# beenotung/bpe-tokenizer

Hardware: NVIDIA B200
Metric: mergeUntil merges/sec (higher is better)
Workload: dtype u32

## Files before the change

### bpe_tokenizer_b200/csrc/bpe_b200.cu

```cuda
#include "../../include/bpe_b200.h"

#include <algorithm>
#include <cstdarg>
#include <cstdio>
#include <cstdlib>
#include <chrono>
#include <cstring>
#include <functional>
#include <string>
#include <unordered_map>
#include <vector>

#include "encode_kernels.cuh"
#include "encode_lanes.cuh"
#include "encode_dp.cuh"
#include "train_kernels.cuh"
#include "mg_kernels.cuh"
#include "round_kernels.cuh"
#include "text_kernels.cuh"

using namespace bpe;

namespace {

// ... 87 lines not shown

struct EncodeScratch {
  DevBuf<int32_t> out_tmp;
  DevBuf<uint32_t> out_len;
  DevBuf<uint64_t> out_off;
  DevBuf<uint32_t> g_tok, g_nxt, g_prv, g_rk, g_sel;
  DevBuf<uint32_t> range_first, tile_sums;
  DevBuf<uint64_t> tile_off;
  DevBuf<uint32_t> flags;
  DevBuf<uint16_t> dp_last;
  DevBuf<unsigned long long> dp_cursor;
};

struct bpe_engine {
  int device = 0;
  int sm_count = 148;
  cudaStream_t stream = nullptr, own_stream = nullptr;
  std::string err;
  bool profiling = false;
  cudaEvent_t ev0 = nullptr, ev1 = nullptr;

  DevBuf<uint32_t> slots;
  uint64_t n_slots = 0;
  std::vector<int64_t> doc_off{0};
  uint64_t live_tokens = 0;

  std::vector<int32_t> h_len16;
  DevBuf<uint32_t> d_len16;
  int32_t n_tokens = 0;

  std::vector<int32_t> h_merges;
  bool mt_dirty = true;
  DevBuf<unsigned long long> d_mt;
  DevBuf<uint32_t> d_minlr;
  uint32_t mt_cap = 0;
  bool lt_dirty = true;
  DevBuf<uint4> d_lt;
  DevBuf<uint2> d_lt_dense;
  DevBuf<uint16_t> d_rule_c;
  uint32_t lt_cap = 0;
  int32_t lt_c_affine = -1;
  bool dp_dirty = true, dp_ok = false;
  DevBuf<unsigned long long> d_dfa;
  DevBuf<uint32_t> d_split;
  DevBuf<uint16_t> d_tok_len, d_shorter;
  bool dp_attr_set = false;
  uint32_t dp_alpha = 0;
  int enc_dp = 0;
  int enc_lmax = 32;
  int enc_lmax_forced = 0;
  int enc_force_old = 0;

  bool index_valid = false;
  uint32_t tbl_cap = 0;
  DevBuf<uint32_t> t_ent;
  DevBuf<uint32_t> u_ent;
  DevBuf<uint32_t> pool;
  DevBuf<DevState> d_st;
  DevState* h_st = nullptr;
  DevBuf<Best> partials;
  DevBuf<uint32_t> partial_keys;
  DevBuf<SiteRec> sites, sites2;
  DevBuf<uint32_t> newslots;
  DevBuf<uint32_t> nd;
  DevBuf<uint32_t> hot;
  bool hot_valid = false;
  uint32_t hot_max_length = 0;
  uint32_t hot_thresh = 0;
  uint32_t hot_limit = 0;
  DevBuf<uint32_t> cands;
  DevBuf<MergeRec> dev_log;
  DevBuf<unsigned long long> barrier;
  int loop_blocks = 0;
  DevBuf<unsigned long long> r_cells;
  DevBuf<uint32_t> r_slotrows, r_lists;
  DevBuf<SiteRec> r_bsites;
  DevBuf<uint4> r_gp;
  DevBuf<uint32_t> r_gk;
  DevBuf<RoundState> r_state;
  DevBuf<unsigned long long> r_gcells;
  DevBuf<uint32_t> r_glists;
  int round_blocks = 0;
  int host_loop = 0;
  int scan_mode = 0;

  int mg_rank = 0, mg_world = 1;
  void* mg_mailbox = nullptr;
  size_t mg_mailbox_bytes = 0;
  void* mg_peer[MG_MAX_WORLD] = {};
  bool mg_connected = false;
  bool mg_counts_global = false;
  uint32_t mg_inbox_stride = 0, mg_tie_cap = 0;
  DevBuf<int32_t> mg_dlt;
  DevBuf<uint32_t> mg_mark, mg_touched, mg_tie_sorted, mg_export_n, mg_newpair;
  int mg_loop_blocks = 0;
  unsigned long long mg_epoch = 0, mg_tie_epoch = 0;

  DevBuf<int32_t> d_cpmap;
  DevBuf<uint32_t> d_firstpos;
  DevBuf<uint8_t> x_text;
  DevBuf<uint32_t> x_tilecnt;
  DevBuf<uint64_t> x_tileoff;
  DevBuf<unsigned long long> x_counts;
  DevBuf<uint32_t> x_doccnt;
  DevBuf<uint64_t> x_docoff;

  DevBuf<int32_t> x_ids, x_out, x_tvi;
  DevBuf<int64_t> x_off, x_ooff, x_ooff2, x_bad;
  DevBuf<unsigned long long> x_flag;
  std::vector<int64_t> h_rel;
  EncodeScratch x_scratch;
  EncodeScratch dev_scratch;
  uint32_t lanes_attr_set = 0;
  cudaStream_t s_in = nullptr, s_out = nullptr;
  cudaEvent_t ev_in[3] = {nullptr, nullptr, nullptr}, ev_done = nullptr, ev_res[2] = {nullptr, nullptr};
  unsigned long long* h_pipe = nullptr;
  PinBuf<int64_t> h_in_off, h_out_off, h_bad;
  int64_t enc_chunk = 128ll << 20;

  DevBuf<int32_t> stage_ids;
  DevBuf<int64_t> stage_off;

  bpe_stats stats{};

  PairTable table() const {
    PairTable t;
    const size_t fs = (TBL_STRIDE == 1) ? (size_t)tbl_cap : 1;
    t.keys.p = t_ent.p;
    t.cnt.p = t_ent.p + fs;
    t.occ_start.p = t_ent.p + 2 * fs;
    t.occ_len.p = t_ent.p + 3 * fs;
    t.occ_fill.p = t_ent.p + 4 * fs;
    t.mask = tbl_cap - 1;
    t.shift = 32 - ilog2(tbl_cap);
    return t;
  }
  int grid(int per_sm = 4) const { return sm_count * per_sm; }
};

namespace {

int fail(bpe_engine* e, int code, const char* fmt, ...) {
  char buf[512];
  va_list ap;
  va_start(ap, fmt);
  vsnprintf(buf, sizeof buf, fmt, ap);
  va_end(ap);
  if (e) e->err = buf;
  return code;
}

#define CK(call)                                                                                              \
  do {                                                                                                        \
    cudaError_t _err = (call);                                                                                \
    if (_err != cudaSuccess)                                                                                  \
      return fail(e, _err == cudaErrorMemoryAllocation ? BPE_E_NOMEM : BPE_E_CUDA, "%s:%d %s: %s", __FILE__, \
                  __LINE__, #call, cudaGetErrorString(_err));                                                 \
  } while (0)

#define CKL()                                \
  do {                                       \
    e->stats.kernel_launches++;              \
    CK(cudaGetLastError());                  \
  } while (0)

#define TRY(call)             \
  do {                        \
    int _rc = (call);         \
    if (_rc != BPE_OK) return _rc; \
  } while (0)

int fetch_state(bpe_engine* e) {
  CK(cudaMemcpyAsync(e->h_st, e->d_st.p, sizeof(DevState), cudaMemcpyDeviceToHost, e->stream));
  CK(cudaStreamSynchronize(e->stream));
  return BPE_OK;
}

int check_dev_err(bpe_engine* e) {
  uint32_t f = e->h_st->err & ~ERR_HOT_OVERFLOW;
  if (!f) return BPE_OK;
  if (f & ERR_POOL_FULL) return fail(e, BPE_E_INTERNAL, "occurrence pool exhausted (flags 0x%x)", f);
  if (f & ERR_MISSING_KEY) return fail(e, BPE_E_INTERNAL, "pair missing from the table (flags 0x%x)", f);
  if (f & ERR_SPAN_OVERFLOW) return fail(e, BPE_E_DOMAIN, "token span exceeds 2^29 positions");
  return fail(e, BPE_E_INTERNAL, "device error flags 0x%x", f);
}

int sync_len16(bpe_engine* e) {
  size_t n = e->h_len16.size();
  CK(e->d_len16.reserve(std::max<size_t>(n + 1024, 4096), 0, e->stream, 2.0));
  if (n) {
    std::vector<uint32_t> tmp(e->h_len16.begin(), e->h_len16.end());
    CK(cudaMemcpyAsync(e->d_len16.p, tmp.data(), n * sizeof(uint32_t), cudaMemcpyHostToDevice, e->stream));
    CK(cudaStreamSynchronize(e->stream));
  }
  return BPE_OK;
}

__global__ void k_init_table(uint4* __restrict__ ent, uint64_t cap) {
  uint64_t stride = (uint64_t)gridDim.x * blockDim.x;
  for (uint64_t i = (uint64_t)blockIdx.x * blockDim.x + threadIdx.x; i < cap; i += stride) {
    ent[2 * i] = make_uint4(EMPTY_KEY, 0u, 0u, 0u);
    ent[2 * i + 1] = make_uint4(0u, 0u, 0u, 0u);
  }
}

int alloc_table(bpe_engine* e, uint32_t cap) {
  CK(e->t_ent.reserve((size_t)cap * (TBL_STRIDE == 1 ? 5 : TBL_STRIDE)));
  e->tbl_cap = cap;
  if (TBL_STRIDE == 1) {
    CK(cudaMemsetAsync(e->t_ent.p, 0xFF, (size_t)cap * 4, e->stream));
    CK(cudaMemsetAsync(e->t_ent.p + cap, 0, (size_t)cap * 16, e->stream));
  } else {
    k_init_table<<<e->grid(8), 256, 0, e->stream>>>(reinterpret_cast<uint4*>(e->t_ent.p), (uint64_t)cap);
    CKL();
  }
  if (e->mg_world > 1) {
    CK(e->mg_dlt.reserve(cap));
    CK(cudaMemsetAsync(e->mg_dlt.p, 0, (size_t)cap * 4, e->stream));
  }
  return BPE_OK;
}

__global__ void k_rehash(PairTable src, PairTable dst, DevState* st) {
  uint32_t cap = src.mask + 1;
  for (uint32_t i = blockIdx.x * blockDim.x + threadIdx.x; i < cap; i += gridDim.x * blockDim.x) {
    uint32_t key = src.keys[i];
    if (key == EMPTY_KEY) continue;
    uint32_t h = (key * 0x9E3779B1u) >> dst.shift;
    for (;;) {
      uint32_t old = atomicCAS(dst.keys + h, EMPTY_KEY, key);
      if (old == EMPTY_KEY) break;
      h = (h + 1) & dst.mask;
    }
    dst.cnt[h] = src.cnt[i];
    dst.occ_start[h] = src.occ_start[i];
    dst.occ_len[h] = src.occ_len[i];
    dst.occ_fill[h] = src.occ_fill[i];
  }
}

int grow_table(bpe_engine* e, uint32_t new_cap) {
  PairTable old = e->table();
  std::swap(e->t_ent, e->u_ent);
  TRY(alloc_table(e, new_cap));
  k_rehash<<<e->grid(), 256, 0, e->stream>>>(old, e->table(), e->d_st.p);
  CKL();
  CK(cudaStreamSynchronize(e->stream));
  e->hot_valid = false;
  return BPE_OK;
}

int build_index(bpe_engine* e) {
  e->index_valid = false;
  e->hot_valid = false;
  if (!e->h_st) CK(cudaHostAlloc((void**)&e->h_st, sizeof(DevState), cudaHostAllocDefault));
  CK(e->d_st.reserve(1));
  CK(e->partials.reserve((size_t)e->grid(8)));
  if (!e->nd.p) CK(e->nd.reserve((size_t)ND_ROWS * ND_STRIDE));
  CK(cudaMemsetAsync(e->nd.p, 0, (size_t)ND_ROWS * ND_STRIDE * 4, e->stream));
  TRY(sync_len16(e));
  uint64_t n = e->n_slots;
  if (n >= 0xFFFFFFF0ull) return fail(e, BPE_E_DOMAIN, "corpus of %llu positions exceeds the 2^32 engine limit", (unsigned long long)n);
  uint64_t pool_need = 3 * n + 1024;
  if (pool_need > 0xFFFFFFF0ull) pool_need = 0xFFFFFFF0ull;
  CK(e->pool.reserve((size_t)pool_need));
  uint64_t t2 = (uint64_t)e->n_tokens * (uint64_t)e->n_tokens;
  uint32_t cap = pow2_at_least(std::min<uint64_t>(std::max<uint64_t>(2 * std::min(n, t2), 1u << 16), 1u << 24));
  {
    if (!e->ev0) {
      CK(cudaEventCreate(&e->ev0));
      CK(cudaEventCreate(&e->ev1));
    }
    CK(cudaEventRecord(e->ev0, e->stream));
  }
  for (;;) {
    TRY(alloc_table(e, cap));
    DevState init{};
    init.live_tokens = e->live_tokens;
    init.tie_pos = ~0ull;
    init.mg_epoch = e->mg_epoch;
    init.mg_tie_epoch = e->mg_tie_epoch;
    CK(cudaMemcpyAsync(e->d_st.p, &init, sizeof init, cudaMemcpyHostToDevice, e->stream));
    CK(cudaStreamSynchronize(e->stream));
    if (n) {
      k_hist<<<e->grid(4), K1_THREADS, 0, e->stream>>>(e->slots.p, (uint32_t)n, e->table(), e->d_st.p);
      CKL();
    }
    TRY(fetch_state(e));
    if (e->h_st->err & ERR_TABLE_FULL) {
      if (cap >= 0x80000000u) return fail(e, BPE_E_NOMEM, "pair table cannot grow further");
      cap <<= 2;
      continue;
    }
    TRY(check_dev_err(e));
    if ((uint64_t)e->h_st->n_keys * 2 > cap && cap < 0x80000000u) {
      cap <<= 1;
      continue;
    }
    break;
  }
  if (n) {
    k_alloc_lists<<<e->grid(4), 256, 0, e->stream>>>(e->table(), e->d_st.p, (uint32_t)e->pool.cap);
    CKL();
    int k1b_per_sm = 8;
    if (const char* v = getenv("BPE_K1B_PER_SM")) k1b_per_sm = std::max(1, std::min(atoi(v), 8));
    k_scatter<<<e->grid(k1b_per_sm), K1_THREADS, 0, e->stream>>>(e->slots.p, (uint32_t)n, e->table(), e->pool.p, e->d_st.p);
    CKL();
  }
  CK(cudaEventRecord(e->ev1, e->stream));
  TRY(fetch_state(e));
  TRY(check_dev_err(e));
  float ms = 0;
  CK(cudaEventElapsedTime(&ms, e->ev0, e->ev1));
  e->stats.ms_index_build += ms;
  e->stats.index_builds++;
  e->index_valid = true;
  e->mg_counts_global = false;
  return BPE_OK;
}

int ensure_index(bpe_engine* e) {
  if (e->index_valid) return BPE_OK;
  return build_index(e);
}

constexpr uint32_t HOT_TARGET = 1u << 15;

int rebuild_hot(bpe_engine* e, uint32_t max_length, bool* any) {
  PairTable t = e->table();
  CK(cudaMemsetAsync(&e->d_st.p->bins[0], 0, sizeof(uint32_t) * 36, e->stream));
  k_count_bins<<<e->grid(4), 256, 0, e->stream>>>(t, e->d_len16.p, max_length, e->d_st.p);
  CKL();
  TRY(fetch_state(e));
  uint64_t acc = 0;
  int pick = 0;
  for (int k = 32; k >= 1; k--) {
    uint64_t nk = e->h_st->bins[k];
    if (acc + nk > HOT_TARGET && acc > 0) break;
    acc += nk;
    if (nk) pick = k;
    if (acc > HOT_TARGET) break;
  }
  *any = pick != 0;
  e->hot_valid = false;
  if (!pick) return BPE_OK;
  int lo = pick;
  while (lo > 1 && e->h_st->bins[lo - 1] == 0) lo--;
  uint32_t thresh = 1u << (lo - 1);
  CK(e->hot.reserve(std::max<size_t>((size_t)acc * 2 + 4096 + 2 * (size_t)BPE_MAX_TOKENS, 1u << 18)));
  e->h_st->hot_n = 0;
  e->h_st->hot_thresh = thresh;
  uint32_t two[2] = {0, thresh};
  CK(cudaMemcpyAsync(&e->d_st.p->hot_n, two, sizeof two, cudaMemcpyHostToDevice, e->stream));
  k_build_hot<<<e->grid(4), 256, 0, e->stream>>>(t, e->d_len16.p, max_length, e->hot.p, (uint32_t)e->hot.cap, e->d_st.p);
  CKL();
  e->hot_thresh = thresh;
  e->hot_limit = (uint32_t)std::min<uint64_t>(std::max<uint64_t>(4ull * HOT_TARGET, 2 * acc + 4096), 0xFFFFFFF0u);
  e->hot_max_length = max_length;
  e->hot_valid = true;
  e->stats.hot_rebuilds++;
  return BPE_OK;
}

int run_argmax(bpe_engine* e, uint32_t max_length, int use_hot) {
  PairTable t = e->table();
  int blocks = use_hot ? e->sm_count : e->grid(4);
  k_argmax<<<blocks, AM_THREADS, 0, e->stream>>>(t, e->d_len16.p, max_length, use_hot, e->hot.p, e->partials.p, e->d_st.p);
  CKL();
  TRY(fetch_state(e));
  TRY(check_dev_err(e));
  if (e->h_st->best_primary && e->h_st->best_mult > 1 && !(use_hot && e->h_st->best_cnt < e->hot_thresh)) {
    uint32_t mult = e->h_st->best_mult;
    CK(e->cands.reserve(std::max<size_t>(mult, 1024), 0, e->stream, 2.0));
    k_collect_cands<<<blocks, 256, 0, e->stream>>>(t, e->d_len16.p, max_length, use_hot, e->hot.p, e->cands.p, (uint32_t)e->cands.cap, e->d_st.p);
    CKL();
    k_tie_break<<<std::min<uint32_t>(mult, (uint32_t)e->grid(4)), 256, 0, e->stream>>>(e->slots.p, (uint32_t)e->n_slots, t, e->pool.p, e->cands.p, e->d_st.p);
    CKL();
    k_tie_finish<<<1, 32, 0, e->stream>>>(t, e->d_st.p);
    CKL();
    TRY(fetch_state(e));
    TRY(check_dev_err(e));
    e->stats.tie_breaks++;
  }
  return BPE_OK;
}

ApplyArgs apply_args(bpe_engine* e) {
  ApplyArgs A;
  A.slots = e->slots.p;
  A.n = (uint32_t)e->n_slots;
  A.t = e->table();
  A.pool = e->pool.p;
  A.st = e->d_st.p;
  A.sites = e->sites.p;
  A.sites_cap = (uint32_t)std::min<size_t>(e->sites.cap, 0xFFFFFFFFu);
  A.newslots = e->newslots.p;
  A.nd = e->nd.p;
  A.newpair = nullptr;
  A.newpair_cap = 0;
  A.new_cap = (uint32_t)std::min<size_t>(e->newslots.cap, 0xFFFFFFFFu);
  A.len16 = e->d_len16.p;
  A.scan_mode = e->scan_mode;
  A.dlt = nullptr;
  A.touched = nullptr;
  A.touched_cap = 0;
  for (int q = 0; q < 8; q++) A.push[q] = nullptr;
  A.push_world = 0;
  A.push_cap = 0;
  return A;
}

int run_apply(bpe_engine* e, uint32_t a, uint32_t b, uint32_t c, uint32_t bound) {
  uint64_t keys_after = (uint64_t)e->h_st->n_keys + std::min<uint64_t>(2ull * bound + 2, 2ull * ((uint64_t)e->n_tokens + 1) + 2);
  if (keys_after * 2 > e->tbl_cap) {
    uint64_t want = keys_after * 5 / 2;
    if (want > 0x80000000ull) want = 0x80000000ull;
    if (keys_after * 2 > pow2_at_least(want)) return fail(e, BPE_E_NOMEM, "pair table cannot grow further");
    TRY(grow_table(e, pow2_at_least(want)));
  }
  uint64_t pool_after = (uint64_t)e->h_st->pool_cursor + 2ull * bound;
  if (pool_after > e->pool.cap) {
    if (pool_after > 0xFFFFFFF0ull) return fail(e, BPE_E_DOMAIN, "occurrence pool exceeds 2^32 cells");
    CK(e->pool.reserve((size_t)pool_after, e->h_st->pool_cursor, e->stream, 1.5));
  }
  CK(e->sites.reserve(std::max<size_t>(bound, 4096), 0, e->stream, 2.0));
  CK(e->newslots.reserve(std::max<size_t>(2ull * bound + 2, 8192), 0, e->stream, 2.0));
  if ((size_t)c + 1 > e->d_len16.cap) CK(e->d_len16.reserve((size_t)c + 1, (size_t)c, e->stream, 2.0));
  PairTable t = e->table();
  uint32_t work = e->scan_mode ? (uint32_t)e->n_slots : bound;
  int blocks = (int)std::min<uint64_t>((uint64_t)e->grid(8), std::max<uint64_t>(1, (work + 255) / 256));
  ApplyArgs A = apply_args(e);
  k_sites<<<blocks, 256, 0, e->stream>>>(A, a, b, c);
  CKL();
  int blocks2 = (int)std::min<uint64_t>((uint64_t)e->grid(8), std::max<uint64_t>(1, (2ull * bound + 255) / 256));
  k_alloc_new<<<blocks2, 256, 0, e->stream>>>(A, c, e->hot_max_length, e->hot_valid ? 1 : 0, e->hot.p, (uint32_t)e->hot.cap, (uint32_t)e->pool.cap);
  CKL();
  int blocks3 = (int)std::min<uint64_t>((uint64_t)e->grid(8), std::max<uint64_t>(1, ((uint64_t)bound + 255) / 256));
  k_apply<<<blocks3, 256, 0, e->stream>>>(A, a, b, c);
  CKL();
  e->h_len16.push_back(e->h_len16[a] + e->h_len16[b]);
  e->h_merges.push_back((int32_t)a);
  e->h_merges.push_back((int32_t)b);
  e->h_merges.push_back((int32_t)c);
  e->mt_dirty = e->lt_dirty = e->dp_dirty = true;
  e->n_tokens++;
  e->stats.merges_applied++;
  return BPE_OK;
}

int ensure_merge_table(bpe_engine* e) {
  if (!e->mt_dirty && e->d_mt.p) return BPE_OK;
  size_t m = e->h_merges.size() / 3;
  uint32_t cap = pow2_at_least(std::max<size_t>(4 * m, 1024));
  std::vector<unsigned long long> h(cap, MT_EMPTY);
  int shift = 32 - ilog2(cap);
  for (size_t r = 0; r < m; r++) {
    uint32_t a = (uint32_t)e->h_merges[3 * r], b = (uint32_t)e->h_merges[3 * r + 1], c = (uint32_t)e->h_merges[3 * r + 2];
    uint32_t key = pair_key(a, b);
    uint32_t i = (key * 0x9E3779B1u) >> shift;
    bool dup = false;
    while (h[i] != MT_EMPTY) {
      if ((uint32_t)(h[i] >> 32) == key) {
        dup = true;
        break;
      }
      i = (i + 1) & (cap - 1);
    }
    if (!dup) h[i] = ((unsigned long long)key << 32) | ((unsigned long long)(uint32_t)r << 16) | c;
  }
  std::vector<uint32_t> minlr((size_t)std::max(e->n_tokens, 1), 0xFFFFFFFFu);
  for (size_t r = 0; r < m; r++) {
    uint32_t a = (uint32_t)e->h_merges[3 * r], b = (uint32_t)e->h_merges[3 * r + 1];
    if (a >= minlr.size() || b >= minlr.size()) return fail(e, BPE_E_INVALID, "merge %zu refers to a token outside the table", r);
    uint32_t rr = (uint32_t)std::min<size_t>(r, 0xFFFE);
    if ((minlr[a] >> 16) > rr) minlr[a] = (minlr[a] & 0xFFFFu) | (rr << 16);
    if ((minlr[b] & 0xFFFFu) > rr) minlr[b] = (minlr[b] & 0xFFFF0000u) | rr;
  }
  CK(e->d_minlr.reserve(minlr.size()));
  CK(cudaMemcpyAsync(e->d_minlr.p, minlr.data(), minlr.size() * 4, cudaMemcpyHostToDevice, e->stream));
  CK(e->d_mt.reserve(cap));
  CK(cudaMemcpyAsync(e->d_mt.p, h.data(), (size_t)cap * 8, cudaMemcpyHostToDevice, e->stream));
  CK(cudaStreamSynchronize(e->stream));
  e->mt_cap = cap;
  e->mt_dirty = false;
  return BPE_OK;
}

struct LaneEnt {
  uint16_t rk = 0xFFFF, c = 0, rs = 0xFFFF, ls = 0xFFFF;
};

int build_lane_entries(bpe_engine* e, const std::vector<int32_t>& merges, int32_t n_tokens, std::unordered_map<uint32_t, LaneEnt>& M,
                       std::vector<uint16_t>& rule_c) {
  size_t m = merges.size() / 3;
  if (m > EL_MAX_RANK + 1) return fail(e, BPE_E_DOMAIN, "merge list too long");
  const int32_t nt = std::max(n_tokens, 1);
  M.clear();
  M.reserve(m * 3 + 16);
  std::vector<int32_t> def_a((size_t)nt, -1), def_b((size_t)nt, -1);
  std::vector<uint8_t> first(m, 0);
  rule_c.assign(std::max<size_t>(m, 1), 0);
  for (size_t r = 0; r < m; r++) {
    int32_t a = merges[3 * r], b = merges[3 * r + 1], c = merges[3 * r + 2];
    if (a < 0 || b < 0 || c < 0 || a >= nt || b >= nt || c >= nt)
      return fail(e, BPE_E_INVALID, "merge %zu refers to a token outside the table", r);
    rule_c[r] = (uint16_t)c;
    if (def_a[c] < 0 && a < c && b < c) {
      def_a[c] = a;
      def_b[c] = b;
    } else if (def_a[c] >= 0 && (def_a[c] != a || def_b[c] != b)) {
      return fail(e, BPE_E_INVALID, "token %d is produced by two different merges", c);
    }
    LaneEnt& x = M[pair_key((uint32_t)a, (uint32_t)b)];
    if (x.rk == 0xFFFF) {
      x.rk = (uint16_t)r;
      x.c = (uint16_t)c;
      first[r] = 1;
    }
  }
  for (size_t r = 0; r < m; r++) {
    if (!first[r]) continue;
    int32_t a = merges[3 * r], b = merges[3 * r + 1];
    for (int32_t u = a;;) {
      LaneEnt& x = M[pair_key((uint32_t)u, (uint32_t)b)];
      if (x.rs > r) x.rs = (uint16_t)r;
      if (def_a[u] < 0) break;
      u = def_b[u];
    }
    for (int32_t w = b;;) {
      LaneEnt& x = M[pair_key((uint32_t)a, (uint32_t)w)];
      if (x.ls > r) x.ls = (uint16_t)r;
      if (def_a[w] < 0) break;
      w = def_a[w];
    }
  }
  return BPE_OK;
}

int ensure_lane_tables(bpe_engine* e) {
  if (!e->lt_dirty && e->d_lt.p) return BPE_OK;
  size_t m = e->h_merges.size() / 3;
  std::unordered_map<uint32_t, LaneEnt> M;
  std::vector<uint16_t> rule_c;
  TRY(build_lane_entries(e, e->h_merges, e->n_tokens, M, rule_c));
  uint32_t cap = pow2_at_least(std::max<size_t>(2 * M.size(), 1024));
  std::vector<uint4> h(cap, make_uint4(EMPTY_KEY, EL_NONE, 0xFFFFFFFFu, 0));
  std::vector<uint2> dense((size_t)EL_DENSE * EL_DENSE, make_uint2(EL_NONE, 0xFFFFFFFFu));
  int shift = 32 - ilog2(cap);
  for (auto& kv : M) {
    uint32_t key = kv.first;
    const LaneEnt& x = kv.second;
    uint32_t y = (uint32_t)x.rk | ((uint32_t)x.c << 16), z = (uint32_t)x.rs | ((uint32_t)x.ls << 16);
    uint32_t a = key >> 16, b = key & 0xFFFFu;
    if (a < (uint32_t)EL_DENSE && b < (uint32_t)EL_DENSE) dense[a * EL_DENSE + b] = make_uint2(y, z);
    uint32_t i = (key * 0x9E3779B1u) >> shift;
    while (h[i].x != EMPTY_KEY) i = (i + 1) & (cap - 1);
    h[i] = make_uint4(key, y, z, 0);
  }
  CK(e->d_lt.reserve(cap));
  CK(cudaMemcpyAsync(e->d_lt.p, h.data(), (size_t)cap * sizeof(uint4), cudaMemcpyHostToDevice, e->stream));
  CK(e->d_lt_dense.reserve(dense.size()));
  CK(cudaMemcpyAsync(e->d_lt_dense.p, dense.data(), dense.size() * sizeof(uint2), cudaMemcpyHostToDevice, e->stream));
  CK(e->d_rule_c.reserve(rule_c.size()));
  CK(cudaMemcpyAsync(e->d_rule_c.p, rule_c.data(), rule_c.size() * sizeof(uint16_t), cudaMemcpyHostToDevice, e->stream));
  CK(cudaStreamSynchronize(e->stream));
  e->lt_cap = cap;
  e->lt_c_affine = m ? (int32_t)rule_c[0] : 0;
  for (size_t r = 0; r < m; r++)
    if ((int64_t)rule_c[r] != (int64_t)rule_c[0] + (int64_t)r) e->lt_c_affine = -1;
  e->lt_dirty = false;
  return BPE_OK;
}

int ensure_dp_tables(bpe_engine* e) {
  if (!e->dp_dirty) return BPE_OK;
  e->dp_dirty = false;
  e->dp_ok = false;
  const size_t m = e->h_merges.size() / 3;
  const int64_t n_tok = e->n_tokens;
  const int64_t A = n_tok - (int64_t)m;
  if (A <= 0 || A > 4096 || n_tok > 0xFFF0) return BPE_OK;
  std::vector<uint32_t> split((size_t)n_tok), off((size_t)n_tok + 1, 0);
  std::vector<uint16_t> tok_len((size_t)n_tok, 1);
  for (int64_t t = 0; t < A; t++) split[(size_t)t] = (uint32_t)t | ((uint32_t)t << 16);
  for (size_t r = 0; r < m; r++) {
    const int64_t a = e->h_merges[3 * r], b = e->h_merges[3 * r + 1], c = e->h_merges[3 * r + 2];
    if (c != A + (int64_t)r || a < 0 || b < 0 || a >= c || b >= c) return BPE_OK;
    const uint32_t L = (uint32_t)tok_len[(size_t)a] + tok_len[(size_t)b];
    if (L > 0xFFF0u) return BPE_OK;
    tok_len[(size_t)c] = (uint16_t)L;
    split[(size_t)c] = (uint32_t)a | ((uint32_t)b << 16);
  }
  for (int64_t t = 0; t < n_tok; t++) off[(size_t)t + 1] = off[(size_t)t] + tok_len[(size_t)t];
  if (off[(size_t)n_tok] > (64u << 20)) return BPE_OK;
  std::vector<uint16_t> text(off[(size_t)n_tok]);
  for (int64_t t = 0; t < A; t++) text[off[(size_t)t]] = (uint16_t)t;
  for (size_t r = 0; r < m; r++) {
    const size_t a = (size_t)e->h_merges[3 * r], b = (size_t)e->h_merges[3 * r + 1], c = (size_t)e->h_merges[3 * r + 2];
    std::copy(text.begin() + off[a], text.begin() + off[a + 1], text.begin() + off[c]);
    std::copy(text.begin() + off[b], text.begin() + off[b + 1], text.begin() + off[c] + tok_len[a]);
  }
  std::unordered_map<uint64_t, uint32_t> child;
  child.reserve(text.size() * 2);
  std::vector<uint16_t> node_tok(1, (uint16_t)DP_NONE);
  std::vector<uint32_t> node_of((size_t)n_tok), parent(1, 0);
  std::vector<uint16_t> pch(1, 0);
  for (int64_t t = 0; t < n_tok; t++) {
    uint32_t v = 0;
    for (uint32_t i = off[(size_t)t]; i < off[(size_t)t + 1]; i++) {
// ... 1960 lines not shown
```

### bpe_tokenizer_b200/csrc/train_kernels.cuh

```cuda
#pragma once
#include "common.cuh"

namespace bpe {

struct DevState {
  uint32_t n_keys;
  uint32_t pool_cursor;
  uint32_t err;
  uint32_t hot_n;
  uint32_t hot_thresh;
  uint32_t n_sites[2];
  uint32_t n_new[2];
  uint32_t n_cand;
  uint32_t blocks_done;
  unsigned long long best_primary;
  uint32_t best_slot;
  uint32_t best_mult;
  uint32_t best_a, best_b, best_cnt;
  uint32_t list_len;
  unsigned long long tie_pos;
  unsigned long long live_tokens;
  unsigned long long _unused_barrier;
  uint32_t n_tokens;
  uint32_t iters_done;
  uint32_t status;
  uint32_t tie_breaks;
  unsigned long long sites_total;
  uint32_t snap_n_keys, snap_pool_cursor, snap_hot_n, snap_err;
  unsigned long long prof_ns[8];
  uint32_t bins[36];
  unsigned long long mg_epoch;
  unsigned long long mg_tie_epoch;
  uint32_t n_touched[2];
  uint32_t n_out;
  uint32_t n_newpair;
  uint32_t mg_abort;
  unsigned long long mg_prof_ns[12];
  alignas(16) uint32_t g_vals[8];
  unsigned long long fine_ns[12];
  unsigned long long bucket_ns[32][4];
};

constexpr uint32_t LOOP_RUNNING = 0, LOOP_DONE = 1, LOOP_NEED_REBUILD = 2, LOOP_NEED_HOST = 3, LOOP_EMPTY = 4,
                   LOOP_ERROR = 5, LOOP_LIMIT = 6;

struct SiteRec {
  uint32_t p;
  uint32_t lpos;
  uint32_t lslot;
  uint32_t rslot;
};

struct MergeRec {
  int32_t a, b, c, reserved;
  long long weight;
};

__device__ __forceinline__ unsigned long long make_primary(uint32_t cnt, uint32_t a, uint32_t b) {
  return ((unsigned long long)cnt << 20) | (unsigned long long)(0xFFFFFu - (a + b));
}

__device__ __forceinline__ uint32_t lane_id() { return threadIdx.x & 31u; }

__global__ void k_ingest_ids(const int32_t* __restrict__ ids, uint32_t* __restrict__ slots, uint64_t n,
                             uint32_t max_id, uint32_t* __restrict__ err) {
  uint64_t i4 = (uint64_t)blockIdx.x * blockDim.x + threadIdx.x;
  uint64_t stride = (uint64_t)gridDim.x * blockDim.x;
  uint64_t n4 = n >> 2;
  bool aligned = ((((uintptr_t)ids) | ((uintptr_t)slots)) & 15) == 0;
  uint32_t bad = 0;
  if (aligned) {
    for (uint64_t i = i4; i < n4; i += stride) {
      int4 v = __ldg(reinterpret_cast<const int4*>(ids) + i);
      bad |= ((uint32_t)v.x >= max_id) | ((uint32_t)v.y >= max_id) | ((uint32_t)v.z >= max_id) | ((uint32_t)v.w >= max_id);
      reinterpret_cast<uint4*>(slots)[i] = make_uint4((uint32_t)v.x, (uint32_t)v.y, (uint32_t)v.z, (uint32_t)v.w);
    }
    for (uint64_t i = (n4 << 2) + i4; i < n; i += stride) {
      uint32_t v = (uint32_t)ids[i];
      bad |= v >= max_id;
      slots[i] = v;
    }
  } else {
    for (uint64_t i = i4; i < n; i += stride) {
      uint32_t v = (uint32_t)ids[i];
      bad |= v >= max_id;
      slots[i] = v;
    }
  }
  if (bad) atomicOr(err, 1u);
}

__global__ void k_validate_ids(const uint32_t* __restrict__ slots, uint64_t n, uint32_t max_id, uint32_t* __restrict__ err) {
  uint64_t stride = (uint64_t)gridDim.x * blockDim.x;
  uint32_t bad = 0;
  for (uint64_t i = (uint64_t)blockIdx.x * blockDim.x + threadIdx.x; i < n; i += stride) bad |= slots[i] >= max_id;
  if (bad) atomicOr(err, 1u);
}

__global__ void k_mark_docstarts(uint32_t* __restrict__ slots, const int64_t* __restrict__ doc_off, int64_t n_docs,
                                 int64_t base) {
  int64_t d = (int64_t)blockIdx.x * blockDim.x + threadIdx.x;
  int64_t stride = (int64_t)gridDim.x * blockDim.x;
  for (; d < n_docs; d += stride) {
    int64_t s = doc_off[d], e = doc_off[d + 1];
    if (e > s) slots[base + s] |= DOCSTART;
  }
}

constexpr int K1_THREADS = 256;
constexpr int K1_SMEM_SLOTS = 2048;
constexpr int K1_MAX_PROBE = 8;
#ifndef BPE_K1B_CHUNK_LOG
#define BPE_K1B_CHUNK_LOG 16
#endif
constexpr uint32_t K1B_CHUNK = 1u << BPE_K1B_CHUNK_LOG;

struct SmemHist {
  uint32_t key[K1_SMEM_SLOTS];
  uint32_t a[K1_SMEM_SLOTS];
  uint32_t b[K1_SMEM_SLOTS];
};

__device__ __forceinline__ int sh_slot(SmemHist& sh, uint32_t key, bool insert) {
  uint32_t h = (key * 0x9E3779B1u) >> (32 - 11);
#pragma unroll 1
  for (int probe = 0; probe < K1_MAX_PROBE; probe++) {
    uint32_t k = sh.key[h];
    if (k == EMPTY_KEY) {
      if (!insert) return -1;
      uint32_t old = atomicCAS(&sh.key[h], EMPTY_KEY, key);
      k = (old == EMPTY_KEY) ? key : old;
    }
    if (k == key) return (int)h;
    h = (h + 1) & (K1_SMEM_SLOTS - 1);
  }
  return -1;
}

__device__ __forceinline__ bool edge_at(const uint32_t* __restrict__ slots, uint32_t n, uint32_t p, uint32_t w,
                                        uint32_t wnext_hint, uint32_t* key, uint32_t* counted) {
  if (!slot_is_id(w)) return false;
  uint32_t a = slot_val(w);
  int b;
  if (slot_is_id(wnext_hint)) {
    b = (wnext_hint & DOCSTART) ? NOTOK : (int)slot_val(wnext_hint);
  } else {
    uint32_t q;
    b = right_token(slots, n, p, &q);
  }
  if (b == NOTOK) return false;
  *key = pair_key(a, (uint32_t)b);
  if (counted) {
    *counted = 1;
    if ((uint32_t)b == a) *counted = (run_left(slots, p, w, (int)a) & 1u) ? 0u : 1u;
  }
  return true;
}

__device__ __forceinline__ void load_group(const uint32_t* __restrict__ slots, uint32_t n, uint32_t g, uint32_t v[5]) {
  uint32_t p0 = g << 2;
  if (p0 + 4 <= n) {
    uint4 q = ld_slots4(slots + p0);
    v[0] = q.x; v[1] = q.y; v[2] = q.z; v[3] = q.w;
  } else {
#pragma unroll
    for (int j = 0; j < 4; j++) v[j] = (p0 + j < n) ? ld_slot(slots + p0 + j) : mk_hole();
  }
  v[4] = (p0 + 4 < n) ? ld_slot(slots + p0 + 4) : (DOCSTART);
}

__global__ void __launch_bounds__(K1_THREADS) k_hist(const uint32_t* __restrict__ slots, uint32_t n, PairTable t,
                                                      DevState* st) {
  __shared__ SmemHist sh;
  for (int i = threadIdx.x; i < K1_SMEM_SLOTS; i += K1_THREADS) {
    sh.key[i] = EMPTY_KEY;
    sh.a[i] = 0;
    sh.b[i] = 0;
  }
  __syncthreads();
  uint32_t n4 = (n + 3) >> 2;
  uint32_t per_block = (n4 + gridDim.x - 1) / gridDim.x;
  uint32_t g_begin = blockIdx.x * per_block;
  uint32_t g_end = min(n4, g_begin + per_block);
  for (uint32_t g = g_begin + threadIdx.x; g < g_end; g += K1_THREADS) {
    uint32_t p0 = g << 2;
    uint32_t v[5];
    load_group(slots, n, g, v);
#pragma unroll
    for (int j = 0; j < 4; j++) {
      uint32_t key, counted;
      if (p0 + j < n && edge_at(slots, n, p0 + j, v[j], v[j + 1], &key, &counted)) {
        int h = sh_slot(sh, key, true);
        if (h >= 0) {
          atomicAdd(&sh.a[h], 1u);
          if (!counted) atomicAdd(&sh.b[h], 1u);
        } else {
          uint32_t gs = tbl_find_or_insert(t, key, &st->n_keys);
          if (gs == NOSLOT) {
            atomicOr(&st->err, ERR_TABLE_FULL);
          } else {
            if (counted) atomicAdd(t.cnt + gs, 1u);
            atomicAdd(t.occ_len + gs, 1u);
          }
        }
      }
    }
  }
  __syncthreads();
  uint32_t n_ins = 0;
  for (int i = threadIdx.x; i < K1_SMEM_SLOTS; i += K1_THREADS) {
    uint32_t key = sh.key[i];
    if (key == EMPTY_KEY) continue;
    bool ins;
    uint32_t gs = tbl_find_or_insert_ex(t, key, &ins);
    if (gs == NOSLOT) {
      atomicOr(&st->err, ERR_TABLE_FULL);
      continue;
    }
    n_ins += ins ? 1u : 0u;
    if (sh.a[i] != sh.b[i]) atomicAdd(t.cnt + gs, sh.a[i] - sh.b[i]);
    if (sh.a[i]) atomicAdd(t.occ_len + gs, sh.a[i]);
  }
#pragma unroll
  for (int o = 16; o > 0; o >>= 1) n_ins += __shfl_xor_sync(0xFFFFFFFFu, n_ins, o);
  if ((threadIdx.x & 31) == 0 && n_ins) atomicAdd(&st->n_keys, n_ins);
}

__global__ void k_alloc_lists(PairTable t, DevState* st, uint32_t pool_cap) {
  uint32_t cap = t.mask + 1;
  for (uint32_t i = blockIdx.x * blockDim.x + threadIdx.x; i < cap; i += gridDim.x * blockDim.x) {
    if (t.keys[i] == EMPTY_KEY) continue;
    uint32_t len = t.occ_len[i];
    t.occ_fill[i] = 0;
    if (len == 0) continue;
    uint32_t start = atomicAdd(&st->pool_cursor, len);
    if (start > pool_cap || len > pool_cap - start) atomicOr(&st->err, ERR_POOL_FULL);
    t.occ_start[i] = start;
  }
}

__global__ void __launch_bounds__(K1_THREADS) k_scatter(const uint32_t* __restrict__ slots, uint32_t n, PairTable t,
                                                         uint32_t* __restrict__ pool, DevState* st) {
  __shared__ SmemHist sh;
  uint32_t n_chunks = (n + K1B_CHUNK - 1) / K1B_CHUNK;
  for (uint32_t chunk = blockIdx.x; chunk < n_chunks; chunk += gridDim.x) {
    for (int i = threadIdx.x; i < K1_SMEM_SLOTS; i += K1_THREADS) {
      sh.key[i] = EMPTY_KEY;
      sh.a[i] = 0;
    }
    __syncthreads();
    uint32_t g_begin = chunk * (K1B_CHUNK >> 2);
    uint32_t g_end = min((n + 3) >> 2, g_begin + (K1B_CHUNK >> 2));
    for (uint32_t g = g_begin + threadIdx.x; g < g_end; g += K1_THREADS) {
      uint32_t p0 = g << 2;
      uint32_t v[5];
      load_group(slots, n, g, v);
#pragma unroll
      for (int j = 0; j < 4; j++) {
        uint32_t key;
        if (p0 + j < n && edge_at(slots, n, p0 + j, v[j], v[j + 1], &key, nullptr)) {
          int h = sh_slot(sh, key, true);
          if (h >= 0) atomicAdd(&sh.a[h], 1u);
        }
      }
    }
    __syncthreads();
    for (int i = threadIdx.x; i < K1_SMEM_SLOTS; i += K1_THREADS) {
      uint32_t key = sh.key[i];
      if (key == EMPTY_KEY) continue;
      uint32_t gs = tbl_find(t, key);
      if (gs == NOSLOT) {
        atomicOr(&st->err, ERR_MISSING_KEY);
        sh.b[i] = NOPOS;
      } else {
        sh.b[i] = t.occ_start[gs] + atomicAdd(t.occ_fill + gs, sh.a[i]);
      }
      sh.a[i] = 0;
    }
    __syncthreads();
    for (uint32_t g = g_begin + threadIdx.x; g < g_end; g += K1_THREADS) {
      uint32_t p0 = g << 2;
      uint32_t v[5];
      load_group(slots, n, g, v);
#pragma unroll
      for (int j = 0; j < 4; j++) {
        uint32_t key;
        if (p0 + j < n && edge_at(slots, n, p0 + j, v[j], v[j + 1], &key, nullptr)) {
          int h = sh_slot(sh, key, false);
          if (h >= 0) {
            uint32_t base = sh.b[h];
            if (base != NOPOS) pool[base + atomicAdd(&sh.a[h], 1u)] = p0 + j;
          } else {
            uint32_t gs = tbl_find(t, key);
            if (gs == NOSLOT) atomicOr(&st->err, ERR_MISSING_KEY);
            else pool[t.occ_start[gs] + atomicAdd(t.occ_fill + gs, 1u)] = p0 + j;
          }
        }
      }
    }
    __syncthreads();
  }
}

struct Best {
  unsigned long long primary;
  uint32_t slot;
  uint32_t mult;
};

__device__ __forceinline__ Best best_merge(Best x, Best y) {
  if (x.primary > y.primary) return x;
  if (y.primary > x.primary) return y;
  Best r;
  r.primary = x.primary;
  r.slot = min(x.slot, y.slot);
  r.mult = x.mult + y.mult;
  return r;
}

__device__ __forceinline__ Best best_warp_reduce(Best v) {
#pragma unroll
  for (int o = 16; o > 0; o >>= 1) {
    Best w;
    w.primary = __shfl_xor_sync(0xFFFFFFFFu, v.primary, o);
    w.slot = __shfl_xor_sync(0xFFFFFFFFu, v.slot, o);
    w.mult = __shfl_xor_sync(0xFFFFFFFFu, v.mult, o);
    v = best_merge(v, w);
  }
  return v;
}

__device__ __forceinline__ Best best_block_reduce(Best v, Best* s_best) {
  v = best_warp_reduce(v);
  __syncthreads();
  if (lane_id() == 0) s_best[threadIdx.x >> 5] = v;
  __syncthreads();
  uint32_t nw = blockDim.x >> 5;
  Best u = (lane_id() < nw) ? s_best[lane_id()] : Best{0ull, NOSLOT, 0};
  u = best_warp_reduce(u);
  return u;
}

__device__ __forceinline__ unsigned long long slot_primary(const PairTable& t, const uint32_t* len16, uint32_t s,
                                                           uint32_t max_length) {
  uint32_t key = t.keys[s];
  if (key == EMPTY_KEY) return 0ull;
  uint32_t c = t.cnt[s];
  if (c == 0) return 0ull;
  uint32_t a = key >> 16, b = key & 0xFFFFu;
  if (max_length && len16[a] + len16[b] > max_length) return 0ull;
  return make_primary(c, a, b);
}

__device__ __forceinline__ unsigned long long slot_primary_k(const PairTable& t, const uint32_t* len16, uint32_t s, uint32_t max_length,
                                                             uint32_t* key_out) {
  uint32_t key = t.keys[s];
  *key_out = key;
  if (key == EMPTY_KEY) return 0ull;
  uint32_t c = t.cnt[s];
  if (c == 0) return 0ull;
  uint32_t a = key >> 16, b = key & 0xFFFFu;
  if (max_length && len16[a] + len16[b] > max_length) return 0ull;
  return make_primary(c, a, b);
}

__device__ __forceinline__ Best argmax_stripe(const PairTable& t, const uint32_t* len16, uint32_t max_length, int use_hot,
                                              const uint32_t* hot, uint32_t n, uint32_t bid, uint32_t nblk) {
  Best mine{0ull, NOSLOT, 0};
  for (uint32_t i = bid * blockDim.x + threadIdx.x; i < n; i += nblk * blockDim.x) {
    uint32_t s = use_hot ? hot[i] : i;
    unsigned long long pr = slot_primary(t, len16, s, max_length);
    if (pr) mine = best_merge(mine, Best{pr, s, 1});
  }
  return mine;
}

__device__ __forceinline__ void publish_best(const PairTable& t, DevState* st, Best u) {
  st->best_primary = u.primary;
  st->best_slot = u.slot;
  st->best_mult = u.mult;
  if (u.primary) {
    uint32_t key = t.keys[u.slot];
    st->best_a = key >> 16;
    st->best_b = key & 0xFFFFu;
    st->best_cnt = t.cnt[u.slot];
    st->list_len = t.occ_len[u.slot];
  } else {
    st->best_a = st->best_b = st->best_cnt = st->list_len = 0;
  }
}

constexpr int AM_THREADS = 256;

__global__ void __launch_bounds__(AM_THREADS) k_argmax(PairTable t, const uint32_t* __restrict__ len16,
                                                        uint32_t max_length, int use_hot,
                                                        const uint32_t* __restrict__ hot, Best* __restrict__ partials,
                                                        DevState* st) {
  __shared__ Best s_best[AM_THREADS / 32];
  __shared__ bool s_last;
  uint32_t n = use_hot ? st->hot_n : (t.mask + 1);
  Best v = best_block_reduce(argmax_stripe(t, len16, max_length, use_hot, hot, n, blockIdx.x, gridDim.x), s_best);
  if (threadIdx.x == 0) {
    partials[blockIdx.x] = v;
    __threadfence();
    uint32_t done = atomicAdd(&st->blocks_done, 1u);
    s_last = (done == gridDim.x - 1);
  }
  __syncthreads();
  if (!s_last) return;
  __threadfence();
  Best w{0ull, NOSLOT, 0};
  for (uint32_t i = threadIdx.x; i < gridDim.x; i += blockDim.x) w = best_merge(w, partials[i]);
  w = best_block_reduce(w, s_best);
  if (threadIdx.x == 0) {
    publish_best(t, st, w);
    st->blocks_done = 0;
    st->n_sites[0] = st->n_sites[1] = 0;
    st->n_new[0] = st->n_new[1] = 0;
    st->n_cand = 0;
    st->tie_pos = ~0ull;
  }
}

__device__ __forceinline__ void phase_collect(const PairTable& t, const uint32_t* len16, uint32_t max_length, int use_hot,
                                              const uint32_t* hot, uint32_t n, unsigned long long best, uint32_t* cands,
                                              uint32_t cand_cap, DevState* st, uint32_t bid, uint32_t nblk) {
  for (uint32_t i = bid * blockDim.x + threadIdx.x; i < n; i += nblk * blockDim.x) {
    uint32_t s = use_hot ? hot[i] : i;
    if (slot_primary(t, len16, s, max_length) == best) {
      uint32_t k = atomicAdd(&st->n_cand, 1u);
      if (k < cand_cap) cands[k] = s;
      else atomicOr(&st->err, ERR_CAND_OVERFLOW);
    }
  }
}

__global__ void k_collect_cands(PairTable t, const uint32_t* __restrict__ len16, uint32_t max_length, int use_hot,
                                const uint32_t* __restrict__ hot, uint32_t* __restrict__ cands, uint32_t cand_cap,
                                DevState* st) {
  uint32_t n = use_hot ? st->hot_n : (t.mask + 1);
  phase_collect(t, len16, max_length, use_hot, hot, n, st->best_primary, cands, cand_cap, st, blockIdx.x, gridDim.x);
}

__device__ __forceinline__ bool counted_occurrence(const uint32_t* slots, uint32_t n, uint32_t p, uint32_t a, uint32_t b) {
  uint32_t w = ld_slot(slots + p);
  if (!slot_is_id(w) || slot_val(w) != a) return false;
  uint32_t q;
  if (right_token(slots, n, p, &q) != (int)b) return false;
  if (a == b && (run_left(slots, p, w, (int)a) & 1u)) return false;
  return true;
}

__device__ __forceinline__ void phase_tie(const uint32_t* slots, uint32_t n, const PairTable& t, const uint32_t* pool,
                                          const uint32_t* cands, uint32_t n_cand, DevState* st, uint32_t* s_max,
                                          uint32_t bid, uint32_t nblk) {
  for (uint32_t c = bid; c < n_cand; c += nblk) {
    uint32_t s = cands[c];
    uint32_t key = t.keys[s];
    uint32_t a = key >> 16, b = key & 0xFFFFu;
    uint32_t start = t.occ_start[s], len = t.occ_len[s];
    uint32_t v = 0;
    for (uint32_t i = threadIdx.x; i < len; i += blockDim.x) {
      uint32_t p = pool[start + i];
      if (counted_occurrence(slots, n, p, a, b)) v = max(v, p + 1);
    }
#pragma unroll
    for (int o = 16; o > 0; o >>= 1) v = max(v, __shfl_xor_sync(0xFFFFFFFFu, v, o));
    __syncthreads();
    if (lane_id() == 0) s_max[threadIdx.x >> 5] = v;
    __syncthreads();
    if (threadIdx.x == 0) {
      uint32_t m = 0;
      for (uint32_t i = 0; i < (blockDim.x >> 5); i++) m = max(m, s_max[i]);
      if (m) atomicMin(&st->tie_pos, ((unsigned long long)(m - 1) << 32) | s);
    }
  }
}

__global__ void __launch_bounds__(256) k_tie_break(const uint32_t* __restrict__ slots, uint32_t n, PairTable t,
                                                    const uint32_t* __restrict__ pool,
                                                    const uint32_t* __restrict__ cands, DevState* st) {
  __shared__ uint32_t s_max[32];
  phase_tie(slots, n, t, pool, cands, st->n_cand, st, s_max, blockIdx.x, gridDim.x);
}

__global__ void k_tie_finish(PairTable t, DevState* st) {
  if (threadIdx.x == 0 && blockIdx.x == 0 && st->tie_pos != ~0ull) {
    uint32_t s = (uint32_t)(st->tie_pos & 0xFFFFFFFFu);
    uint32_t key = t.keys[s];
    st->best_slot = s;
    st->best_a = key >> 16;
    st->best_b = key & 0xFFFFu;
    st->best_cnt = t.cnt[s];
    st->list_len = t.occ_len[s];
  }
}

__global__ void k_lookup_pair(PairTable t, uint32_t a, uint32_t b, DevState* st) {
  if (threadIdx.x == 0 && blockIdx.x == 0) {
    uint32_t s = tbl_find(t, pair_key(a, b));
    st->best_slot = s;
    st->best_a = a;
    st->best_b = b;
    st->best_cnt = (s == NOSLOT) ? 0 : t.cnt[s];
    st->list_len = (s == NOSLOT) ? 0 : t.occ_len[s];
    st->n_sites[0] = st->n_sites[1] = 0;
    st->n_new[0] = st->n_new[1] = 0;
    st->n_cand = 0;
  }
}

__global__ void k_count_bins(PairTable t, const uint32_t* __restrict__ len16, uint32_t max_length, DevState* st) {
  __shared__ uint32_t s_bins[36];
  if (threadIdx.x < 36) s_bins[threadIdx.x] = 0;
  __syncthreads();
  uint32_t cap = t.mask + 1;
  for (uint32_t i = blockIdx.x * blockDim.x + threadIdx.x; i < cap; i += gridDim.x * blockDim.x) {
    unsigned long long pr = slot_primary(t, len16, i, max_length);
    if (pr) atomicAdd(&s_bins[32 - __clz((uint32_t)(pr >> 20))], 1u);
  }
  __syncthreads();
  if (threadIdx.x < 36 && s_bins[threadIdx.x]) atomicAdd(&st->bins[threadIdx.x], s_bins[threadIdx.x]);
}

__global__ void k_build_hot(PairTable t, const uint32_t* __restrict__ len16, uint32_t max_length,
                            uint32_t* __restrict__ hot, uint32_t hot_cap, DevState* st) {
  uint32_t cap = t.mask + 1;
  uint32_t thresh = st->hot_thresh;
  for (uint32_t i = blockIdx.x * blockDim.x + threadIdx.x; i < cap; i += gridDim.x * blockDim.x) {
    unsigned long long pr = slot_primary(t, len16, i, max_length);
    if (pr && (uint32_t)(pr >> 20) >= thresh) {
      uint32_t k = atomicAdd(&st->hot_n, 1u);
      if (k < hot_cap) hot[k] = i;
      else atomicOr(&st->err, ERR_HOT_OVERFLOW);
    }
  }
}

struct ApplyArgs {
  uint32_t* slots;
  uint32_t n;
  PairTable t;
  uint32_t* pool;
  DevState* st;
  SiteRec* sites;
  uint32_t sites_cap;
  uint32_t* newslots;
  uint32_t new_cap;
  uint32_t* len16;
  int scan_mode;
  int32_t* dlt;
  uint32_t* touched;
  uint32_t touched_cap;
  uint32_t* nd;
  uint32_t* newpair;
  uint32_t newpair_cap;
  unsigned long long* push[8];
  int push_world;
  uint32_t push_cap;
};

constexpr uint32_t ND_STRIDE = 56320;
enum { ND_L_LEN = 0, ND_L_CNT, ND_R_LEN, ND_R_CNT, ND_L_SLOT, ND_R_SLOT, ND_ROWS };
constexpr uint32_t NOTOKV = 0xFFFFFFFFu;

constexpr uint32_t ERR_TOUCH_OVERFLOW = 128u, ERR_PEER_TIMEOUT = 256u, ERR_INBOX_OVERFLOW = 512u, ERR_PEER = 1024u;

__device__ __forceinline__ unsigned long long now_ns();
__device__ __forceinline__ void prefetch_l1(const void* p) { asm volatile("prefetch.global.L1 [%0];" ::"l"(p)); }
__device__ __forceinline__ void prefetch_l2(const void* p) { asm volatile("prefetch.global.L2 [%0];" ::"l"(p)); }
__device__ __forceinline__ void prefetch_pair(const PairTable& t, uint32_t key) {
  uint32_t h = tbl_hash(t, key);
  prefetch_l1(t.keys + h);
  prefetch_l2(t.cnt + h);
  prefetch_l2(t.occ_len + h);
}

__device__ __forceinline__ void cnt_delta_warp(const ApplyArgs& A, bool has, uint32_t s, uint32_t key, int32_t d, uint32_t par) {
  const uint32_t lane = lane_id();
  if (A.push_world) {
    uint32_t m = __ballot_sync(0xFFFFFFFFu, has);
    if (!m) return;
    uint32_t base = 0;
    int src = __ffs(m) - 1;
    if ((int)lane == src) base = atomicAdd(&A.st->n_out, (uint32_t)__popc(m));
    base = __shfl_sync(0xFFFFFFFFu, base, src);
    if (has) {
      uint32_t k = base + __popc(m & ((1u << lane) - 1u));
      if (k < A.push_cap) {
        unsigned long long rec = ((unsigned long long)key << 32) | (uint32_t)d;
        for (int q = 0; q < A.push_world; q++) A.push[q][k] = rec;
      } else {
        atomicOr(&A.st->err, ERR_INBOX_OVERFLOW);
      }
    }
  } else if (A.dlt) {
    bool first = has && atomicAdd(A.dlt + s, d) == 0;
    uint32_t m = __ballot_sync(0xFFFFFFFFu, first);
    if (!m) return;
    uint32_t base = 0;
    int src = __ffs(m) - 1;
// ... 809 lines not shown
```

Before: 68700.

## Stage scatter positions in shared memory and write pool lists contiguously

k_scatter now computes a block-wide exclusive prefix over the per-key histogram counts, stages each chunk's occurrence offsets as 16-bit values in shared memory grouped by key, then writes them to the global pool in a flat pass. Each global write is located by a binary search over the prefix, so consecutive threads write contiguous runs instead of scattered atomic-indexed stores. The block grows to 1024 threads with dynamic shared memory, the chunk shrinks to 32K entries, and blocks per SM come from the occupancy API. The trade-off is extra shared memory, more barriers and a binary search per output element, and likely lower occupancy. This only affects index build, so its effect on merge throughput depends on how often the index is rebuilt.

After: 71720 (median of 6 runs). +4.4%, better.

```diff
diff --git a/bpe_tokenizer_b200/csrc/bpe_b200.cu b/bpe_tokenizer_b200/csrc/bpe_b200.cu
--- a/bpe_tokenizer_b200/csrc/bpe_b200.cu
+++ b/bpe_tokenizer_b200/csrc/bpe_b200.cu
@@ -413,9 +413,11 @@
   if (n) {
     k_alloc_lists<<<e->grid(4), 256, 0, e->stream>>>(e->table(), e->d_st.p, (uint32_t)e->pool.cap);
     CKL();
-    int k1b_per_sm = 8;
-    if (const char* v = getenv("BPE_K1B_PER_SM")) k1b_per_sm = std::max(1, std::min(atoi(v), 8));
-    k_scatter<<<e->grid(k1b_per_sm), K1_THREADS, 0, e->stream>>>(e->slots.p, (uint32_t)n, e->table(), e->pool.p, e->d_st.p);
+    int k1b_per_sm = 0;
+    CK(cudaFuncSetAttribute(k_scatter, cudaFuncAttributeMaxDynamicSharedMemorySize, (int)K1B_SMEM_BYTES));
+    CK(cudaOccupancyMaxActiveBlocksPerMultiprocessor(&k1b_per_sm, k_scatter, K1B_THREADS, K1B_SMEM_BYTES));
+    if (k1b_per_sm < 1) return fail(e, BPE_E_CUDA, "k_scatter does not fit on an SM");
+    k_scatter<<<e->grid(k1b_per_sm), K1B_THREADS, K1B_SMEM_BYTES, e->stream>>>(e->slots.p, (uint32_t)n, e->table(), e->pool.p, e->d_st.p);
     CKL();
   }
   CK(cudaEventRecord(e->ev1, e->stream));
diff --git a/bpe_tokenizer_b200/csrc/train_kernels.cuh b/bpe_tokenizer_b200/csrc/train_kernels.cuh
--- a/bpe_tokenizer_b200/csrc/train_kernels.cuh
+++ b/bpe_tokenizer_b200/csrc/train_kernels.cuh
@@ -111,15 +111,26 @@
 constexpr int K1_SMEM_SLOTS = 2048;
 constexpr int K1_MAX_PROBE = 8;
 #ifndef BPE_K1B_CHUNK_LOG
-#define BPE_K1B_CHUNK_LOG 16
+#define BPE_K1B_CHUNK_LOG 15
 #endif
+static_assert(BPE_K1B_CHUNK_LOG >= 10 && BPE_K1B_CHUNK_LOG <= 16, "k_scatter stages 16-bit offsets within a chunk");
 constexpr uint32_t K1B_CHUNK = 1u << BPE_K1B_CHUNK_LOG;
+constexpr int K1B_THREADS = 1024;
+static_assert(K1_SMEM_SLOTS % K1B_THREADS == 0 && K1B_THREADS % 32 == 0, "the prefix gives every thread whole slots");
 
 struct SmemHist {
   uint32_t key[K1_SMEM_SLOTS];
   uint32_t a[K1_SMEM_SLOTS];
   uint32_t b[K1_SMEM_SLOTS];
 };
+
+struct SmemScatter {
+  SmemHist h;
+  uint32_t start[K1_SMEM_SLOTS + 1];
+  uint32_t warp_sum[K1B_THREADS / 32];
+  uint16_t stage[K1B_CHUNK];
+};
+constexpr size_t K1B_SMEM_BYTES = sizeof(SmemScatter);
 
 __device__ __forceinline__ int sh_slot(SmemHist& sh, uint32_t key, bool insert) {
   uint32_t h = (key * 0x9E3779B1u) >> (32 - 11);
@@ -239,19 +250,24 @@
   }
 }
 
-__global__ void __launch_bounds__(K1_THREADS) k_scatter(const uint32_t* __restrict__ slots, uint32_t n, PairTable t,
-                                                         uint32_t* __restrict__ pool, DevState* st) {
-  __shared__ SmemHist sh;
-  uint32_t n_chunks = (n + K1B_CHUNK - 1) / K1B_CHUNK;
+__global__ void __launch_bounds__(K1B_THREADS) k_scatter(const uint32_t* __restrict__ slots, uint32_t n, PairTable t,
+                                                          uint32_t* __restrict__ pool, DevState* st) {
+  extern __shared__ __align__(16) unsigned char k1b_smem[];
+  SmemScatter& sh = *reinterpret_cast<SmemScatter*>(k1b_smem);
+  constexpr int PER = K1_SMEM_SLOTS / K1B_THREADS;
+  constexpr int WARPS = K1B_THREADS / 32;
+  const uint32_t lane = lane_id(), warp = threadIdx.x >> 5;
+  const uint32_t n_chunks = (n + K1B_CHUNK - 1) / K1B_CHUNK;
   for (uint32_t chunk = blockIdx.x; chunk < n_chunks; chunk += gridDim.x) {
-    for (int i = threadIdx.x; i < K1_SMEM_SLOTS; i += K1_THREADS) {
-      sh.key[i] = EMPTY_KEY;
-      sh.a[i] = 0;
+    for (int i = threadIdx.x; i < K1_SMEM_SLOTS; i += K1B_THREADS) {
+      sh.h.key[i] = EMPTY_KEY;
+      sh.h.a[i] = 0;
     }
     __syncthreads();
-    uint32_t g_begin = chunk * (K1B_CHUNK >> 2);
-    uint32_t g_end = min((n + 3) >> 2, g_begin + (K1B_CHUNK >> 2));
-    for (uint32_t g = g_begin + threadIdx.x; g < g_end; g += K1_THREADS) {
+    const uint32_t c0 = chunk * K1B_CHUNK;
+    const uint32_t g_begin = c0 >> 2;
+    const uint32_t g_end = min((n + 3) >> 2, g_begin + (K1B_CHUNK >> 2));
+    for (uint32_t g = g_begin + threadIdx.x; g < g_end; g += K1B_THREADS) {
       uint32_t p0 = g << 2;
       uint32_t v[5];
       load_group(slots, n, g, v);
@@ -259,26 +275,57 @@
       for (int j = 0; j < 4; j++) {
         uint32_t key;
         if (p0 + j < n && edge_at(slots, n, p0 + j, v[j], v[j + 1], &key, nullptr)) {
-          int h = sh_slot(sh, key, true);
-          if (h >= 0) atomicAdd(&sh.a[h], 1u);
+          int h = sh_slot(sh.h, key, true);
+          if (h >= 0) atomicAdd(&sh.h.a[h], 1u);
         }
       }
     }
     __syncthreads();
-    for (int i = threadIdx.x; i < K1_SMEM_SLOTS; i += K1_THREADS) {
-      uint32_t key = sh.key[i];
-      if (key == EMPTY_KEY) continue;
-      uint32_t gs = tbl_find(t, key);
-      if (gs == NOSLOT) {
-        atomicOr(&st->err, ERR_MISSING_KEY);
-        sh.b[i] = NOPOS;
-      } else {
-        sh.b[i] = t.occ_start[gs] + atomicAdd(t.occ_fill + gs, sh.a[i]);
-      }
-      sh.a[i] = 0;
-    }
+    const int i0 = threadIdx.x * PER;
+    uint32_t cnt[PER], sum = 0;
+#pragma unroll
+    for (int e = 0; e < PER; e++) {
+      cnt[e] = sh.h.a[i0 + e];
+      sum += cnt[e];
+    }
+    uint32_t inc = sum;
+#pragma unroll
+    for (int o = 1; o < 32; o <<= 1) {
+      uint32_t y = __shfl_up_sync(0xFFFFFFFFu, inc, o);
+      if (lane >= (uint32_t)o) inc += y;
+    }
+    if (lane == 31) sh.warp_sum[warp] = inc;
     __syncthreads();
-    for (uint32_t g = g_begin + threadIdx.x; g < g_end; g += K1_THREADS) {
+    if (warp == 0) {
+      uint32_t w = lane < (uint32_t)WARPS ? sh.warp_sum[lane] : 0u, wi = w;
+#pragma unroll
+      for (int o = 1; o < 32; o <<= 1) {
+        uint32_t y = __shfl_up_sync(0xFFFFFFFFu, wi, o);
+        if (lane >= (uint32_t)o) wi += y;
+      }
+      if (lane < (uint32_t)WARPS) sh.warp_sum[lane] = wi - w;
+    }
+    __syncthreads();
+    uint32_t run = sh.warp_sum[warp] + inc - sum;
+#pragma unroll
+    for (int e = 0; e < PER; e++) {
+      const int i = i0 + e;
+      sh.start[i] = run;
+      if (cnt[e]) {
+        uint32_t gs = tbl_find(t, sh.h.key[i]);
+        if (gs == NOSLOT) {
+          atomicOr(&st->err, ERR_MISSING_KEY);
+          sh.h.b[i] = NOPOS;
+        } else {
+          sh.h.b[i] = t.occ_start[gs] + atomicAdd(t.occ_fill + gs, cnt[e]);
+        }
+      }
+      sh.h.a[i] = run;
+      run += cnt[e];
+    }
+    if (threadIdx.x == K1B_THREADS - 1) sh.start[K1_SMEM_SLOTS] = run;
+    __syncthreads();
+    for (uint32_t g = g_begin + threadIdx.x; g < g_end; g += K1B_THREADS) {
       uint32_t p0 = g << 2;
       uint32_t v[5];
       load_group(slots, n, g, v);
@@ -286,10 +333,9 @@
       for (int j = 0; j < 4; j++) {
         uint32_t key;
         if (p0 + j < n && edge_at(slots, n, p0 + j, v[j], v[j + 1], &key, nullptr)) {
-          int h = sh_slot(sh, key, false);
+          int h = sh_slot(sh.h, key, false);
           if (h >= 0) {
-            uint32_t base = sh.b[h];
-            if (base != NOPOS) pool[base + atomicAdd(&sh.a[h], 1u)] = p0 + j;
+            sh.stage[atomicAdd(&sh.h.a[h], 1u)] = (uint16_t)(p0 + j - c0);
           } else {
             uint32_t gs = tbl_find(t, key);
             if (gs == NOSLOT) atomicOr(&st->err, ERR_MISSING_KEY);
@@ -297,6 +343,16 @@
           }
         }
       }
+    }
+    __syncthreads();
+    const uint32_t total = sh.start[K1_SMEM_SLOTS];
+    for (uint32_t k = threadIdx.x; k < total; k += K1B_THREADS) {
+      uint32_t s = 0;
+#pragma unroll
+      for (uint32_t half = K1_SMEM_SLOTS / 2; half; half >>= 1)
+        if (sh.start[s + half] <= k) s += half;
+      const uint32_t base = sh.h.b[s];
+      if (base != NOPOS) pool[base + (k - sh.start[s])] = c0 + sh.stage[k];
     }
     __syncthreads();
   }
```
